# nannau/DoWnGAN

Hardware: AMD Instinct MI355X
Metric: train-step samples/sec (G+D+GP) (higher is better)
Workload: dtype bf16

## Files before the change

### downgan_amd/_lib.py

```python
from __future__ import annotations

import ctypes as C
import os

_HERE = os.path.dirname(os.path.abspath(__file__))
LIB_PATH = os.environ.get("DG_LIB_OVERRIDE") or os.path.join(_HERE, "csrc", "libdowngan_hip.so")

DG_F32, DG_BF16 = 0, 1
STATUS = {0: "DG_OK", -1: "DG_ERR_BAD_SHAPE", -2: "DG_ERR_BAD_DTYPE", -3: "DG_ERR_BAD_ARG", -4: "DG_ERR_LAUNCH"}


class Epilogue(C.Structure):
    _fields_ = [("bias", C.c_void_p), ("has_act", C.c_int), ("act_slope", C.c_float),
                ("r1", C.c_void_p), ("ldr1", C.c_int64), ("s1", C.c_float),
                ("r2", C.c_void_p), ("ldr2", C.c_int64), ("s2", C.c_float),
                ("mask", C.c_void_p), ("ldmask", C.c_int64), ("mask_slope", C.c_float),
                ("accumulate", C.c_int), ("mask_bits", C.c_void_p), ("out_bits", C.c_void_p),
                ("mask_c0", C.c_int), ("mask_last", C.c_int), ("out_q", C.c_void_p), ("out_qs", C.c_void_p), ("ldqs", C.c_int64),
                ("out_u", C.c_void_p), ("out_ue", C.c_void_p), ("skip_y", C.c_int), ("out_amax", C.c_void_p)]


class ConvGeom(C.Structure):
    _fields_ = [("dtype", C.c_int), ("N", C.c_int), ("H", C.c_int), ("W", C.c_int),
                ("Cin", C.c_int), ("Cout", C.c_int), ("stride", C.c_int), ("cin_real", C.c_int), ("pixel_shuffle", C.c_int),
# ... 102 lines not shown
                ("thr", (C.c_float * OBJ_MAX_THR) * HIST_MAX_OUT)]


class DistmapSpec(C.Structure):
    _fields_ = [("speed_u", C.c_int), ("speed_v", C.c_int), ("nthr", C.c_int), ("nring", C.c_int), ("cutoff", C.c_int),
                ("scale", C.c_float * EOF_MAX_C), ("offset", C.c_float * EOF_MAX_C),
                ("thr", (C.c_float * DIST_MAX_THR) * HIST_MAX_OUT)]


class TemporalSpec(C.Structure):
    _fields_ = [("speed_u", C.c_int), ("speed_v", C.c_int), ("nthr", C.c_int), ("ndur", C.c_int), ("nlag", C.c_int),
                ("nbins", C.c_int), ("below", C.c_int * TEMPORAL_MAX_THR), ("lag", C.c_int * TEMPORAL_MAX_LAGS),
                ("scale", C.c_float * EOF_MAX_C), ("offset", C.c_float * EOF_MAX_C),
                ("thr", (C.c_float * TEMPORAL_MAX_THR) * HIST_MAX_OUT), ("lo", (C.c_float * TEMPORAL_MAX_LAGS) * HIST_MAX_OUT),
                ("inv_w", (C.c_float * TEMPORAL_MAX_LAGS) * HIST_MAX_OUT)]


MINMAX_PARTS = 256
_vp, _i, _i64, _f = C.c_void_p, C.c_int, C.c_int64, C.c_float
_PROTOS = {
    "dg_conv3x3_fwd": [C.POINTER(ConvGeom), C.POINTER(Epilogue), _vp, _vp, _vp, _vp],
    "dg_conv3x3_dgrad": [C.POINTER(ConvGeom), C.POINTER(Epilogue), _vp, _vp, _vp, _vp],
    "dg_conv3x3_wgrad": [C.POINTER(ConvGeom), _vp, _vp, _vp, _vp, _vp],
    "dg_conv3x3_wgrad_dense": [_vp, _i, _vp, _vp, _vp, _vp, _vp],
    "dg_conv3x3_wgrad_f8": [C.POINTER(ConvGeom), _vp, _vp, _vp, _vp, _vp, _vp],
    "dg_exp_from_amax": [_vp, _i, _i, _vp, _vp],
    "dg_conv3x3_wgrad_dense_f8": [C.POINTER(ConvGeom), _i, _vp, _vp, _vp, _vp, _vp, _vp],
    "dg_gather_gemm": [C.POINTER(GGDesc), C.POINTER(Epilogue), _vp, _vp, _vp, _vp],
    "dg_conv3x3_plan": [C.POINTER(ConvGeom), _i, C.POINTER(GGDesc)],
    "dg_last_conv_kernels": [],
    "dg_last_wgrad_kernel": [],
    "dg_conv3x3_dgrad_launches": [C.POINTER(ConvGeom)],
    "dg_conv3x3_dgrad_stream_eligible": [C.POINTER(ConvGeom), C.POINTER(Epilogue)],
    "dg_set_s2_dgrad_stream": [C.c_int],
    "dg_colsum": [_i, _vp, _i64, _i64, _i64, _i64, _i, _vp, _vp],
    "dg_colsum_multi": [_i, _vp, _i64, _i64, _i, _i, _vp, _vp],
    "dg_repack_conv_weights": [_i, _i, _vp, _vp, _i, _i, _vp],
    "dg_repack_dense_dgrad": [_i, _vp, _i, _i, _vp, _vp],
    "dg_wgrad_unswap": [_vp, _vp, _i, _i, _vp],
    "dg_linear_fwd": [_i, _vp, _i64, _vp, _i64, _vp, _i, _i, _i, _i64, _vp],
    "dg_linear_dx": [_i, _i, _vp, _i, _vp, _i64, _vp, _i64, _vp, _i64, _f, _i, _i, _i64, _vp],
    "dg_linear_dw": [_i, _vp, _i, _vp, _i64, _vp, _i64, _i, _i, _i64, _vp],
    "dg_linear_dw_wide": [_i, _vp, _i, _vp, _i64, _vp, _i64, _i, _i, _i64, _i, _vp],
    "dg_bias_act": [_i, _vp, _i, _vp, _vp, _i, _i, _i, _i, _f, _vp, _i, _f, _vp],
    "dg_mask_mul": [_i, _vp, _i64, _vp, _i64, _i64, _i, _f, _vp],
    "dg_axpby": [_i, _vp, _i64, _vp, _i64, _f, _vp, _i64, _f, _i64, _i, _vp],
    "dg_gp_interp": [_i, _vp, _vp, _vp, _vp, _i, _i64, _vp],
    "dg_gp_interp_c2": [_i, _vp, _vp, _i64, _vp, _vp, _vp, _vp, _i, _i64, _vp],
    "dg_scale_rows_c2": [_i, _vp, _i64, _vp, _vp, _i, _i64, _vp],
    "dg_sumsq_rows": [_i, _vp, _i, _i64, _vp, _vp],
    "dg_gp_finish": [_vp, _i, _i, _f, _f, _vp, _vp, _vp],
    "dg_scale_rows": [_i, _vp, _vp, _vp, _i, _i64, _vp],
    "dg_l1": [_i, _vp, _i64, _vp, _i64, _i64, _i, _vp, _vp, _i64, _f, _vp, _i64, _vp],
    "dg_sqdiff": [_i, _vp, _i64, _vp, _i64, _i64, _i, _vp, _vp],
    "dg_sum_strided": [_vp, _i, _i, _f, _vp, _vp],
    "dg_fill_col": [_vp, _i, _i, _i, _f, _vp],
    "dg_adam": [_vp, _vp, _vp, _vp, _vp, _i64, _f, _f, _f, _f, _i, _f, _vp],
    "dg_nchw_to_nhwc": [_i, _vp, _vp, _i, _i, _i, _i, _i, _vp],
    "dg_nhwc_to_nchw": [_i, _vp, _i64, _vp, _i, _i, _i, _i, _vp],
    "dg_cast": [_i, _vp, _vp, _i64, _vp],
    "dg_minmax_partial": [_i, _vp, _i64, _i64, _i, _vp, _vp],
    "dg_minmax_finish": [_vp, _i, _vp, _vp],
    "dg_normalise_planar": [_i, _vp, _i, _i, _i, _i64, _i, _vp, _vp, _vp],
    "dg_ssim_level": [_vp, _vp, _i, _i, _i, C.POINTER(SsimParams), _vp, _vp],
    "dg_avgpool2": [_vp, _vp, _i, _i, _i, _vp],
    "dg_msssim_finish": [_vp, _i, _i, C.POINTER(MsssimCombine), _vp, _vp],
    "dg_div_vort_sums": [_i, _vp, _i64, _vp, _i64, _i, _i, _i, _vp, _vp],
# ... 127 lines not shown
```

### downgan_amd/csrc/conv_plan.hip

```cpp
#include "gg_common.h"

thread_local int g_last_kinds = 0;

static int gg_validate(const dg_gg_desc* d, bool f8 = false, bool compact_src = false) {
  if (d->dtype != DG_F32 && d->dtype != DG_BF16) return DG_ERR_BAD_DTYPE;
  const int epc = f8 ? 16 : d->dtype == DG_F32 ? 4 : 8;
  if (d->N <= 0 || d->Hs <= 0 || d->Ws <= 0 || d->Hg <= 0 || d->Wg <= 0 || d->Hd <= 0 || d->Wd <= 0) return DG_ERR_BAD_SHAPE;
  if (d->Cred <= 0 || d->Cred % 8 || d->Nout <= 0 || d->Nout % 16) return DG_ERR_BAD_SHAPE;
  if (d->ntaps < 1 || d->ntaps > 9) return DG_ERR_BAD_SHAPE;
  if ((compact_src ? d->lds % 2 || d->lds < 2 : d->lds % epc) || d->ldd % 4 || d->ldw % epc) return DG_ERR_BAD_SHAPE;
  for (int t = 0; t < d->ntaps; ++t) {
    if (d->tap_dy[t] < -1 || d->tap_dy[t] > 1 || d->tap_dx[t] < -1 || d->tap_dx[t] > 1) return DG_ERR_BAD_ARG;
    if (d->tap_w[t] < 0 || d->tap_w[t] > 8) return DG_ERR_BAD_ARG;
  }
  if (d->src_ps && ((d->Cred / 4) % 8)) return DG_ERR_BAD_SHAPE;
  if (d->dst_ps && ((d->Nout / 4) % 16)) return DG_ERR_BAD_SHAPE;
  if ((long long)d->N * d->Hg * d->Wg >= (1ll << 31)) return DG_ERR_BAD_SHAPE;
  if (d->dst_ps) {
    if (2 * d->Hg > d->Hd || 2 * d->Wg > d->Wd) return DG_ERR_BAD_SHAPE;
  } else {
    if ((d->Hg - 1) * d->dy_mul + d->dy_off >= d->Hd || (d->Wg - 1) * d->dx_mul + d->dx_off >= d->Wd) return DG_ERR_BAD_SHAPE;
    if (d->dy_off < 0 || d->dx_off < 0 || d->dy_mul < 1 || d->dx_mul < 1) return DG_ERR_BAD_SHAPE;
  }
  return DG_OK;
// ... 147 lines not shown
  }
  int nd = 0;
  const int st = g->stride;
  for (int ph = 0; ph < st; ++ph)
    for (int pw = 0; pw < st; ++pw) {
      dg_gg_desc d{};
      d.dtype = g->dtype; d.N = g->N; d.Hs = Ho; d.Ws = Wo; d.Cred = g->Cout; d.lds = g->ldy;
      d.src_ps = g->pixel_shuffle;
      d.Hg = g->H / st; d.Wg = g->W / st; d.sy_mul = 1; d.sx_mul = 1;
      d.ntaps = 0;
      for (int r = 0; r < 3; ++r) {
        if ((ph + 1 - r) % st) continue;
        for (int s = 0; s < 3; ++s) {
          if ((pw + 1 - s) % st) continue;
          d.tap_dy[d.ntaps] = (ph + 1 - r) / st; d.tap_dx[d.ntaps] = (pw + 1 - s) / st;
          d.tap_w[d.ntaps] = r * 3 + s;
          ++d.ntaps;
        }
      }
      d.Nout = g->Cin; d.ldw = 9ll * g->Cout;
      d.Hd = g->H; d.Wd = g->W; d.ldd = g->ldx;
      d.dy_mul = d.dx_mul = st; d.dy_off = ph; d.dx_off = pw; d.dst_ps = 0;
      out[nd++] = d;
    }
  return nd;
}

extern "C" int dg_conv3x3_fwd(const dg_conv_geom* g, const dg_epilogue* ep, const void* x, const void* w_fwd,
                              void* y, void* stream) {
  dg_gg_desc d[4];
  g_last_kinds = 0;
  int n = dg_conv3x3_plan(g, 0, d);
  if (n < 0) return n;
  const bool small = g->cin_real > 0 && g->cin_real <= 2 && g->stride == 1 && !g->pixel_shuffle;
  return gather_gemm_impl(&d[0], ep, x, w_fwd, y, stream, small);
}

static bool seg_dgrad_desc(const dg_gg_desc* d, int n, dg_gg_desc* out) {
  const int epc = d[0].dtype == DG_F32 ? 4 : 8;
  if (n != 4 || d[0].src_ps || d[0].dst_ps || (d[0].Cred / epc) % 8 || d[0].Nout <= 64 || d[0].Hg < 8 || d[0].Wg < 8) return false;
  if (d[0].ntaps != 1 || d[1].ntaps != 2 || d[2].ntaps != 2 || d[3].ntaps != 4) return false;
  if (!gg_halo_row_step_ok(d[0].Ws, d[0].lds, d[0].dtype, 1)) return false;
  *out = d[3];
  out->ntaps = 0;
  for (int c = 0; c < 4; ++c) {
    if (d[c].dy_off != (c >> 1) || d[c].dx_off != (c & 1) || d[c].dy_mul != 2 || d[c].dx_mul != 2) return false;
    for (int t = 0; t < d[c].ntaps; ++t, ++out->ntaps) {
      out->tap_dy[out->ntaps] = d[c].tap_dy[t]; out->tap_dx[out->ntaps] = d[c].tap_dx[t]; out->tap_w[out->ntaps] = d[c].tap_w[t];
    }
  }
  return out->ntaps == 9;
}

extern "C" int dg_conv3x3_dgrad(const dg_conv_geom* g, const dg_epilogue* ep, const void* dy, const void* w_dgrad,
                                void* dx, void* stream) {
  if (g && g->Cin % 16) return DG_ERR_BAD_SHAPE;
  dg_gg_desc d[4];
  g_last_kinds = 0;
  int n = dg_conv3x3_plan(g, 1, d);
  if (n < 0) return n;
  if (s2dgrad_stream_mode() && s2dgrad_stream_eligible(g, ep))
    return s2dgrad_stream_launch(g, ep, dy, w_dgrad, dx, reinterpret_cast<hipStream_t>(stream));
  dg_gg_desc ds;
  if (seg_dgrad_desc(d, n, &ds)) return gather_gemm_impl(&ds, ep, dy, w_dgrad, dx, stream, false, nullptr, true);
  for (int i = 0; i < n; ++i) {
    int rc = dg_gather_gemm(&d[i], ep, dy, w_dgrad, dx, stream);
// ... 9 lines not shown
  int n = dg_conv3x3_plan(g, 0, d);
  if (n < 0) return n;
  d[0].lds = q->ldxq;
  return gather_gemm_impl(&d[0], ep, q->xq, q->wq, y, stream, false, q);
}

extern "C" int dg_conv3x3_dgrad_f8(const dg_conv_geom* g, const dg_epilogue* ep, const dg_f8_operands* q, void* dx, void* stream) {
  if (!q || !g || g->dtype != DG_BF16 || g->pixel_shuffle || g->Cout % 128 || g->Cin % 16) return DG_ERR_BAD_SHAPE;
  dg_gg_desc d[4];
  g_last_kinds = 0;
  int n = dg_conv3x3_plan(g, 1, d);
  if (n < 0) return n;
  dg_gg_desc ds;
  if (seg_dgrad_desc(d, n, &ds) && ds.Cred % 128 == 0) {
    ds.lds = q->ldxq;
    return gather_gemm_impl(&ds, ep, q->xq, q->wq, dx, stream, false, q, true);
  }
  for (int i = 0; i < n; ++i) {
    d[i].lds = q->ldxq;
    int rc = gather_gemm_impl(&d[i], ep, q->xq, q->wq, dx, stream, false, q);
    if (rc) return rc;
  }
  return DG_OK;
}

extern "C" int dg_last_conv_kernels(void) { return g_last_kinds; }

extern "C" int dg_conv3x3_dgrad_stream_eligible(const dg_conv_geom* g, const dg_epilogue* ep) {
  const int rc = geom_validate(g);
  if (rc) return rc;
  return s2dgrad_stream_eligible(g, ep) ? 1 : 0;
}

extern "C" int dg_conv3x3_dgrad_launches(const dg_conv_geom* g) {
  dg_gg_desc d[4], ds;
  const int n = dg_conv3x3_plan(g, 1, d);
  if (n < 0) return n;
  return seg_dgrad_desc(d, n, &ds) ? 1 : n;
}
```

### downgan_amd/csrc/gg_common.h

```cpp
#pragma once
#include "dg_internal.h"

#include <stdlib.h>
#include <type_traits>


extern thread_local int g_last_kinds;

struct GGArgs {
  const void* x; const void* w; void* y;
  const float* bias; const void* r1; const void* r2; const void* mask;
  const void* mask_bits; void* out_bits;
  void* out_q; void* out_qs;
  void* out_u; const unsigned char* out_ue;
  int no_y;
  unsigned* out_amax;
  int ldqs, qs_shift;
  long long ldx, ldw, ldy, ldr1, ldr2, ldmask;
  int M, Hg, Wg, Hs, Ws;
  int cch, kchunks, Cred, ntaps;
  int sy_mul, sx_mul;
  unsigned long long tap_lo; unsigned tap_hi;
  int Nout, Hd, Wd, dy_mul, dx_mul, dy_off, dx_off;
  int src_ps, dst_ps, cps_src_chunks, cps_dst;
// ... 482 lines not shown
      case 2328: run(std::integral_constant<int, 2328>{}, htag); break;
      case 2336: run(std::integral_constant<int, 2336>{}, htag); break;
      case 258: run(std::integral_constant<int, 258>{}, htag); break;
      case 261: run(std::integral_constant<int, 261>{}, htag); break;
      case 2306: run(std::integral_constant<int, 2306>{}, htag); break;
      case 2309: run(std::integral_constant<int, 2309>{}, htag); break;
      case 4353: run(std::integral_constant<int, 4353>{}, htag); break;
      case 4354: run(std::integral_constant<int, 4354>{}, htag); break;
      case 4357: run(std::integral_constant<int, 4357>{}, htag); break;
      case 6402: run(std::integral_constant<int, 6402>{}, htag); break;
      case 6405: run(std::integral_constant<int, 6405>{}, htag); break;
      default: run(std::integral_constant<int, -1>{}, htag); break;
    }
  };
  dispatch(std::integral_constant<int, 0>{});
  EPI_STAMP(2);
  if constexpr (NH == 2) dispatch(std::integral_constant<int, 1>{});
  EPI_STAMP(3);
#undef EPI_STAMP
}

struct F8Args { const unsigned char* xs; const unsigned char* ws; int ldxs; };

int gg_launch_rows(GGArgs& a, int dtype, hipStream_t st);
bool gg_regroup_taps_by_plane(GGArgs& a);
bool gg_halo_row_step_ok(long long Ws, long long ldx, int dtype, int mult);
int gg_launch_halo(GGArgs& a, int dtype, int N, bool s2, bool ps, int nw, hipStream_t st);
int gg_launch_halo_f8(GGArgs& a, const F8Args& f, int N, bool s2, int nw, hipStream_t st);
int gg_launch_halo16(GGArgs& a, int dtype, int N, hipStream_t st);
int gg_launch_im2col(GGArgs& a, int dtype, hipStream_t st);
bool s2dgrad_stream_eligible(const dg_conv_geom* g, const dg_epilogue* ep);
int s2dgrad_stream_mode();
int s2dgrad_stream_launch(const dg_conv_geom* g, const dg_epilogue* ep, const void* dy, const void* w, void* dx, hipStream_t st);
```

### include/downgan_hip.h

```cpp
#ifndef DOWNGAN_HIP_H
#define DOWNGAN_HIP_H

#include <stddef.h>
#include <stdint.h>

#ifdef __cplusplus
extern "C" {
#endif

#define DG_F32 0
#define DG_BF16 1

typedef enum dg_status {
  DG_OK = 0,
  DG_ERR_BAD_SHAPE = -1,
  DG_ERR_BAD_DTYPE = -2,
  DG_ERR_BAD_ARG = -3,
  DG_ERR_LAUNCH = -4
} dg_status;

typedef struct dg_epilogue {
  const float* bias;
  int has_act;
  float act_slope;
// ... 47 lines not shown
                     const void* w_dgrad, void* dx, void* stream);

int dg_conv3x3_wgrad(const dg_conv_geom* g, const void* x, const void* dy, float* dw, float* db,
                     void* stream);

int dg_conv3x3_wgrad_dense(const dg_conv_geom* g, int nconv, const void* x, const void* dy,
                           float* const* dw, float* const* db, void* stream);

int dg_conv3x3_wgrad_f8(const dg_conv_geom* g, const void* xq, const void* ex, const void* dyq, const void* ey, float* dw,
                        void* stream);

int dg_conv3x3_wgrad_dense_f8(const dg_conv_geom* g, int nconv, const void* xq, const void* ex, const void* dyq, const void* ey,
                              float* const* dw, void* stream);

int dg_colsum(int dtype, const void* dy, int64_t rows_outer, int64_t ld_outer, int64_t rows_inner,
              int64_t ld, int C, float* db, void* stream);

int dg_colsum_multi(int dtype, const void* dy, int64_t rows, int64_t ld, int C, int nseg, float* const* db, void* stream);

int dg_gather_gemm(const dg_gg_desc* d, const dg_epilogue* ep, const void* x, const void* w, void* y,
                   void* stream);

int dg_last_conv_kernels(void);

int dg_last_wgrad_kernel(void);

int dg_conv3x3_plan(const dg_conv_geom* g, int kind, dg_gg_desc* out);

int dg_conv3x3_dgrad_launches(const dg_conv_geom* g);

int dg_conv3x3_dgrad_stream_eligible(const dg_conv_geom* g, const dg_epilogue* ep);

int dg_set_s2_dgrad_stream(int on);

int dg_repack_conv_weights(int dtype, int kind, const float* master, void* dst, int CoutP, int CinP,
                           void* stream);
int dg_repack_dense_dgrad(int dtype, const float* const* masters, int nconv, int F, void* dst, void* stream);
int dg_wgrad_unswap(const float* tmp, float* dw, int CoutP, int CinP, void* stream);


int dg_linear_fwd(int dtype, const void* x, int64_t ldx, const void* w, int64_t ldw, float* y,
                  int ldy, int B, int O, int64_t K, void* stream);
int dg_linear_dx(int dtype, int out_dtype, const float* dy, int ldo, const void* w, int64_t ldw,
                 void* dx, int64_t lddx, const void* mask, int64_t ldmask, float mask_slope, int B,
                 int O, int64_t K, void* stream);
int dg_linear_dw(int dtype, const float* dy, int ldo, const void* x, int64_t ldx, float* dw,
                 int64_t lddw, int B, int O, int64_t K, void* stream);
int dg_linear_dw_wide(int dtype, const float* dy, int ldo, const void* x, int64_t ldx, float* dw,
                      int64_t lddw, int B, int O, int64_t K, int accumulate, void* stream);


int dg_bias_act(int out_dtype, const float* in, int ldi, const float* bias, void* out, int ldo,
                int rows, int C, int has_act, float slope, const void* mask, int ldmask,
                float mask_slope, void* stream);
int dg_mask_mul(int dtype, void* u, int64_t ldu, const void* y, int64_t ldy, int64_t rows, int C,
                float slope, void* stream);
int dg_axpby(int dtype, void* out, int64_t ldo, const void* x, int64_t ldx, float a, const void* y,
             int64_t ldy, float b, int64_t rows, int C, void* stream);
int dg_gp_interp(int dtype, const void* real, const void* fake, const float* alpha, void* xhat,
                 int B, int64_t per_img, void* stream);
int dg_gp_interp_c2(int dtype, const void* real, const void* fake, int64_t ld, const float* alpha,
                    void* xhat_c, void* real_c, void* fake_c, int B, int64_t pix_per_img, void* stream);
int dg_scale_rows_c2(int dtype, const void* g, int64_t ld, const float* coef, void* out_c, int B,
                     int64_t pix_per_img, void* stream);
int dg_sumsq_rows(int dtype, const void* g, int B, int64_t per_img, float* ss, void* stream);
int dg_gp_finish(const float* ss, int B, int B_global, float gp_lambda, float weight, float* coef,
// ... 283 lines not shown
```

Baseline: 74.25.

## Add persistent warp-specialized streaming kernel for stride-2 128-channel conv forward

```diff
diff --git a/downgan_amd/_lib.py b/downgan_amd/_lib.py
--- a/downgan_amd/_lib.py
+++ b/downgan_amd/_lib.py
@@ -159,6 +159,8 @@
     "dg_conv3x3_dgrad_launches": [C.POINTER(ConvGeom)],
     "dg_conv3x3_dgrad_stream_eligible": [C.POINTER(ConvGeom), C.POINTER(Epilogue)],
     "dg_set_s2_dgrad_stream": [C.c_int],
+    "dg_conv3x3_fwd_stream_eligible": [C.POINTER(ConvGeom), C.POINTER(Epilogue)],
+    "dg_set_s2_fwd_stream": [C.c_int],
     "dg_colsum": [_i, _vp, _i64, _i64, _i64, _i64, _i, _vp, _vp],
     "dg_colsum_multi": [_i, _vp, _i64, _i64, _i, _i, _vp, _vp],
     "dg_repack_conv_weights": [_i, _i, _vp, _vp, _i, _i, _vp],
diff --git a/downgan_amd/csrc/conv_plan.hip b/downgan_amd/csrc/conv_plan.hip
--- a/downgan_amd/csrc/conv_plan.hip
+++ b/downgan_amd/csrc/conv_plan.hip
@@ -203,6 +203,8 @@
   g_last_kinds = 0;
   int n = dg_conv3x3_plan(g, 0, d);
   if (n < 0) return n;
+  if (s2fwd_stream_mode() && s2fwd_stream_eligible(g, ep))
+    return s2fwd_stream_launch(g, ep, x, w_fwd, y, reinterpret_cast<hipStream_t>(stream));
   const bool small = g->cin_real > 0 && g->cin_real <= 2 && g->stride == 1 && !g->pixel_shuffle;
   return gather_gemm_impl(&d[0], ep, x, w_fwd, y, stream, small);
 }
@@ -278,6 +280,12 @@
   return s2dgrad_stream_eligible(g, ep) ? 1 : 0;
 }
 
+extern "C" int dg_conv3x3_fwd_stream_eligible(const dg_conv_geom* g, const dg_epilogue* ep) {
+  const int rc = geom_validate(g);
+  if (rc) return rc;
+  return s2fwd_stream_eligible(g, ep) ? 1 : 0;
+}
+
 extern "C" int dg_conv3x3_dgrad_launches(const dg_conv_geom* g) {
   dg_gg_desc d[4], ds;
   const int n = dg_conv3x3_plan(g, 1, d);
diff --git a/downgan_amd/csrc/conv_s2fwd.hip b/downgan_amd/csrc/conv_s2fwd.hip
--- /dev/null
+++ b/downgan_amd/csrc/conv_s2fwd.hip
@@ -0,0 +1,306 @@
+#include "gg_common.h"
+
+#ifndef S2F_ABL
+#define S2F_ABL 0
+#endif
+
+namespace {
+
+constexpr int NT = 512;
+constexpr int PITCH = 288;
+constexpr int ODD_PIX = 17, EVEN_PIX = 16;
+constexpr int EVEN_OFF = ODD_PIX * PITCH;
+constexpr int RING_ROW = (ODD_PIX + EVEN_PIX) * PITCH;
+constexpr int ROW_PIECES = RING_ROW / 16;
+constexpr int NSLOT = 14;
+constexpr int PF = 4;
+static_assert(2 * PF + 5 <= NSLOT, "the requested rows must not land on rows still being read");
+constexpr int NDMA = 5;
+constexpr int HAND_OFF = NSLOT * RING_ROW;
+constexpr int HAND_SLOT = 4 * 64 * 32;
+constexpr int MASK_OFF = HAND_OFF + 2 * HAND_SLOT;
+constexpr int MASK_SLOT = 16 * 16;
+constexpr int LDS_BYTES = MASK_OFF + 2 * MASK_SLOT;
+
+struct S2FArgs {
+  const char* x; const char* w; char* y;
+  char* bits;
+  float slope;
+  int H, W, Ho, Wo;
+  int nstrips, nitems, trips;
+};
+
+__device__ __forceinline__ __amdgpu_buffer_rsrc_t uniform_rsrc(const char* p) {
+  const unsigned long long b = (unsigned long long)p;
+  const unsigned long long u = ((unsigned long long)(unsigned)__builtin_amdgcn_readfirstlane((int)(unsigned)(b >> 32)) << 32) |
+                               (unsigned)__builtin_amdgcn_readfirstlane((int)(unsigned)b);
+  return __builtin_amdgcn_make_buffer_rsrc((void*)u, 0, (int)DG_OOB_OFF, 0x00020000);
+}
+
+template <int EP, bool HEAD>
+__device__ __forceinline__ void s2f_run(const S2FArgs& a, char* lds) {
+  constexpr int NTAP = HEAD ? 5 : 4;
+  const int tid = threadIdx.x, lane = tid & 63, q = (tid >> 6) & 3;
+  const int l15 = lane & 15, g = lane >> 4;
+
+  u32x4_t wr[NTAP * 8];
+  {
+    constexpr int TWH[5] = {4, 3, 5, 1, 7}, TWT[4] = {0, 2, 6, 8};
+#pragma unroll
+    for (int t = 0; t < NTAP; ++t)
+#pragma unroll
+      for (int cb = 0; cb < 2; ++cb)
+#pragma unroll
+        for (int kk = 0; kk < 2; ++kk)
+#pragma unroll
+          for (int j = 0; j < 2; ++j) {
+            const int n = 32 * q + 8 * (l15 >> 2) + 4 * j + (l15 & 3);
+            const int tw = HEAD ? TWH[t] : TWT[t];
+            wr[((t * 2 + cb) * 2 + kk) * 2 + j] =
+                *reinterpret_cast<const u32x4_t*>(a.w + ((long long)n * 1152 + tw * 128 + 64 * cb + 32 * kk + 8 * g) * 2);
+          }
+#pragma unroll
+    for (int i = 0; i < NTAP * 8; ++i) asm volatile("" : "+v"(wr[i]));
+  }
+  const char* const fb0 = lds + l15 * PITCH + g * 16;
+  auto wrap = [](int v) { return v >= NSLOT ? v - NSLOT : v; };
+  auto frag = [&](int slot, int s, int cb, int kk) {
+    return *reinterpret_cast<const uint4*>(fb0 + slot * RING_ROW + (s == 1 ? EVEN_OFF : s == 2 ? PITCH : 0) + cb * 128 + kk * 64);
+  };
+  auto tap = [&](int t, int cb, int slot, int s, f32x4_t (&acc)[2]) {
+#pragma unroll
+    for (int kk = 0; kk < 2; ++kk) {
+      const uint4 b = frag(slot, s, cb, kk);
+#pragma unroll
+      for (int j = 0; j < 2; ++j) {
+        if (S2F_ABL & 4) acc[j][0] += __uint_as_float(b.x ^ wr[((t * 2 + cb) * 2 + kk) * 2 + j][0]);
+        else Mma<bf16_t>::run(__builtin_bit_cast(uint4, wr[((t * 2 + cb) * 2 + kk) * 2 + j]), b, acc[j]);
+      }
+    }
+  };
+  char* const hand = lds + HAND_OFF + q * (64 * 32) + lane * 32;
+
+  if constexpr (HEAD) {
+    const int hw = __builtin_amdgcn_readfirstlane(tid >> 6) - 4;
+    int dsrc[NDMA], ddst[NDMA];
+    unsigned dpad = 0, dfirst = 0;
+#pragma unroll
+    for (int m = 0; m < NDMA; ++m) {
+      int i = hw + 4 * m;
+      if (i > 18) i = 18;
+      ddst[m] = i < 18 ? i * 1024 : 2 * RING_ROW - 1024;
+      const int P = ddst[m] / 16 + lane, rs = P >= ROW_PIECES ? 1 : 0, Pr = P - ROW_PIECES * rs, ps = Pr / 18, c = Pr - 18 * ps;
+      const int pi = ps < ODD_PIX ? 2 * ps : 2 * (ps - ODD_PIX) + 1;
+      dsrc[m] = (rs * a.W + pi - 1) * 256 + c * 16;
+      if (c >= 16) dpad |= 1u << m;
+      if (pi == 0) dfirst |= 1u << m;
+    }
+    const int ring_m0 = __builtin_amdgcn_readfirstlane((int)(unsigned long long)((__attribute__((address_space(3))) char*)lds));
+    const int htid = tid - 256;
+
+    for (int trip = 0; trip < a.trips; ++trip) {
+      const int item = (int)blockIdx.x + trip * (int)gridDim.x;
+      if (item >= a.nitems) break;
+      const int img = item / a.nstrips, x0 = (item - img * a.nstrips) * 16;
+      typedef int i32x4h_t __attribute__((ext_vector_type(4)));
+      i32x4h_t rs4;
+      {
+        const unsigned long long xb = (unsigned long long)(a.x + (long long)img * a.H * a.W * 256);
+        rs4[0] = __builtin_amdgcn_readfirstlane((int)(unsigned)xb);
+        rs4[1] = __builtin_amdgcn_readfirstlane((int)(unsigned)(xb >> 32) & 0xffff);
+        rs4[2] = (int)DG_OOB_OFF;
+        rs4[3] = 0x00020000;
+      }
+      unsigned doff[NDMA];
+#pragma unroll
+      for (int m = 0; m < NDMA; ++m)
+        doff[m] = (((dpad >> m) & 1u) || (x0 == 0 && ((dfirst >> m) & 1u))) ? DG_OOB_OFF : (unsigned)(dsrc[m] + 2 * x0 * 256);
+      auto request_pair = [&](int row, int slot) {
+        const bool ok = row < a.H && !(S2F_ABL & 2);
+        const unsigned ro = (unsigned)row * (unsigned)a.W * 256u;
+#pragma unroll
+        for (int m = 0; m < NDMA; ++m) {
+          const unsigned off = ok ? doff[m] + ro : DG_OOB_OFF;
+          asm volatile("s_mov_b32 m0, %0\n\ts_nop 0\n\tbuffer_load_dwordx4 %1, %2, 0 offen lds"
+                       :: "s"(ring_m0 + slot * RING_ROW + ddst[m]), "v"(off), "s"(rs4) : "memory");
+        }
+      };
+      asm volatile("s_waitcnt vmcnt(0)" ::: "memory");
+#pragma unroll
+      for (int z = 0; z < 3; ++z)
+        if (htid + 256 * z < ROW_PIECES) *reinterpret_cast<uint4*>(lds + (NSLOT - 1) * RING_ROW + (htid + 256 * z) * 16) = uint4{0u, 0u, 0u, 0u};
+      if (x0 == 0 && htid < NSLOT * 16) *reinterpret_cast<uint4*>(lds + (htid >> 4) * RING_ROW + (htid & 15) * 16) = uint4{0u, 0u, 0u, 0u};
+#pragma unroll
+      for (int d = 0; d < PF; ++d) request_pair(2 * d, 2 * d);
+      asm volatile("s_waitcnt vmcnt(%0)" :: "n"(NDMA * (PF - 1)) : "memory");
+      __syncthreads();
+      int sk = 0;
+      for (int k = 0; k <= a.Ho; ++k) {
+        request_pair(2 * (k + PF), wrap(sk + 2 * PF));
+        if (k < a.Ho) {
+          const int sM = wrap(sk + NSLOT - 1), sP = sk + 1;
+          f32x4_t acc[2] = {f32x4_t{0.f, 0.f, 0.f, 0.f}, f32x4_t{0.f, 0.f, 0.f, 0.f}};
+#pragma unroll
+          for (int cb = 0; cb < 2; ++cb) tap(0, cb, sk, 1, acc);
+#pragma unroll
+          for (int cb = 0; cb < 2; ++cb) { tap(1, cb, sk, 0, acc); tap(2, cb, sk, 2, acc); }
+#pragma unroll
+          for (int cb = 0; cb < 2; ++cb) { tap(3, cb, sM, 1, acc); tap(4, cb, sP, 1, acc); }
+          char* const h = hand + (k & 1) * HAND_SLOT;
+          *reinterpret_cast<f32x4_t*>(h) = acc[0];
+          *reinterpret_cast<f32x4_t*>(h + 16) = acc[1];
+        }
+        asm volatile("s_waitcnt vmcnt(%0)" :: "n"(NDMA * (PF - 1)) : "memory");
+        __syncthreads();
+        sk = wrap(sk + 2);
+      }
+    }
+  } else {
+    const bool mwave = EP == 1 && __builtin_amdgcn_readfirstlane(tid >> 6) == 0;
+    const unsigned st_lane = (unsigned)(l15 * 256 + 64 * q + 16 * g);
+
+    for (int trip = 0; trip < a.trips; ++trip) {
+      const int item = (int)blockIdx.x + trip * (int)gridDim.x;
+      if (item >= a.nitems) break;
+      const int img = item / a.nstrips, x0 = (item - img * a.nstrips) * 16;
+      const __amdgpu_buffer_rsrc_t rY = uniform_rsrc(a.y + (long long)img * a.Ho * a.Wo * 256);
+      const __amdgpu_buffer_rsrc_t rB = uniform_rsrc(a.bits + (long long)img * a.Ho * a.Wo * 16);
+      const unsigned mfill_off = (mwave && lane < 16) ? (unsigned)((x0 + lane) * 16) : DG_OOB_OFF;
+      auto fetch_mask = [&](int R) {
+        return __builtin_amdgcn_raw_buffer_load_b128(rB, R < a.Ho ? mfill_off + (unsigned)R * (unsigned)a.Wo * 16u : DG_OOB_OFF, 0, 0);
+      };
+      const char* const mrd = lds + MASK_OFF + l15 * 16 + 4 * q + g;
+      u32x4_t ms0 = {0u, 0u, 0u, 0u}, ms1 = {0u, 0u, 0u, 0u};
+      if (mwave) ms0 = fetch_mask(0);
+      __syncthreads();
+
+      auto step = [&](int k, int sk, const u32x4_t& mstaged, u32x4_t& mnxt) __attribute__((always_inline)) {
+        if (mwave) mnxt = fetch_mask(k + 1);
+        if (k > 0) {
+          const int R = k - 1;
+          const char* const h = hand + (R & 1) * HAND_SLOT;
+          f32x4_t acc[2] = {*reinterpret_cast<const f32x4_t*>(h), *reinterpret_cast<const f32x4_t*>(h + 16)};
+          unsigned mb = 0;
+          if (EP == 1) mb = *reinterpret_cast<const unsigned char*>(mrd + (R & 1) * MASK_SLOT);
+          const int sM = wrap(sk + NSLOT - 3), sP = wrap(sk + NSLOT - 1);
+#pragma unroll
+          for (int cb = 0; cb < 2; ++cb) {
+            tap(0, cb, sM, 0, acc); tap(1, cb, sM, 2, acc); tap(2, cb, sP, 0, acc); tap(3, cb, sP, 2, acc);
+          }
+          float v[8] = {acc[0][0], acc[0][1], acc[0][2], acc[0][3], acc[1][0], acc[1][1], acc[1][2], acc[1][3]};
+          const unsigned pix = (unsigned)R * (unsigned)a.Wo + (unsigned)x0;
+          if (EP == 0) {
+            if (a.slope >= 0.f && a.slope <= 1.f) {
+              typedef float f32x2_t __attribute__((ext_vector_type(2)));
+              const f32x2_t sl2 = {a.slope, a.slope};
+#pragma unroll
+              for (int e = 0; e < 8; e += 2) {
+                const f32x2_t p = f32x2_t{v[e], v[e + 1]} * sl2;
+                v[e] = __builtin_fmaxf(v[e], p[0]); v[e + 1] = __builtin_fmaxf(v[e + 1], p[1]);
+              }
+            } else {
+#pragma unroll
+              for (int e = 0; e < 8; ++e) v[e] = leaky(v[e], a.slope);
+            }
+          } else {
+            unsigned sh = mb << 24;
+            const float one = 1.f;
+#pragma unroll
+            for (int e = 7; e >= 0; --e) {
+              float f;
+              asm("v_add_co_u32_e32 %1, vcc, %1, %1\n\tv_cndmask_b32_e32 %0, %2, %3, vcc" : "=&v"(f), "+v"(sh) : "v"(a.slope), "v"(one) : "vcc");
+              v[e] *= f;
+            }
+          }
+          u32x4_t t;
+#pragma unroll
+          for (int e = 0; e < 4; ++e) t[e] = pack_bf16x2(v[2 * e], v[2 * e + 1]);
+          __builtin_amdgcn_raw_buffer_store_b128(t, rY, (S2F_ABL & 1) ? DG_OOB_OFF : pix * 256u + st_lane, 0, 0);
+          if (EP == 0) {
+            unsigned ob = 0;
+#pragma unroll
+            for (int e = 7; e >= 0; --e)
+              asm("v_cmp_lt_f32_e32 vcc, 0, %1\n\tv_addc_co_u32_e32 %0, vcc, %0, %0, vcc" : "+v"(ob) : "v"(v[e]) : "vcc");
+            ob <<= 8 * g;
+            ob |= (unsigned)__shfl_xor((int)ob, 16, 64);
+            ob |= (unsigned)__shfl_xor((int)ob, 32, 64);
+            __builtin_amdgcn_raw_buffer_store_b32(ob, rB, (g == 0 && !(S2F_ABL & 1)) ? (pix + (unsigned)l15) * 16u + 4u * q : DG_OOB_OFF, 0, 0);
+          }
+        }
+        if (mwave && lane < 16) *reinterpret_cast<uint4*>(lds + MASK_OFF + (k & 1) * MASK_SLOT + lane * 16) = __builtin_bit_cast(uint4, mstaged);
+        __syncthreads();
+      };
+      int sk = 0;
+      for (int k = 0; k <= a.Ho; k += 2) {
+        step(k, sk, ms0, ms1);
+        sk = wrap(sk + 2);
+        if (k + 1 <= a.Ho) { step(k + 1, sk, ms1, ms0); sk = wrap(sk + 2); }
+      }
+    }
+  }
+}
+
+std::atomic<int> g_s2f_stream{1};
+std::atomic<int> g_cus{0};
+
+}
+
+template <int EP>
+__global__ __launch_bounds__(NT, 1) void s2fwd_stream_kernel(const S2FArgs a) {
+  extern __shared__ __attribute__((aligned(16))) char s2f_lds[];
+  if (__builtin_amdgcn_readfirstlane(threadIdx.x >> 6) < 4) s2f_run<EP, false>(a, s2f_lds);
+  else s2f_run<EP, true>(a, s2f_lds);
+}
+
+bool s2fwd_stream_eligible(const dg_conv_geom* g, const dg_epilogue* ep) {
+  if (!g || !ep || g->dtype != DG_BF16 || g->stride != 2 || g->pixel_shuffle) return false;
+  if (g->N <= 0 || g->H <= 0 || g->W <= 0 || ((g->H | g->W) & 1)) return false;
+  if (g->Cin != 128 || g->Cout != 128 || g->ldx != 128 || g->ldy != 128) return false;
+  if ((g->W / 2) % 16) return false;
+  if (!gg_halo_row_step_ok(g->W, g->ldx, g->dtype, 2)) return false;
+  if ((long long)g->H * g->W * 256 >= (1ll << 31)) return false;
+  if (ep->bias || ep->r1 || ep->r2 || ep->mask || ep->accumulate || ep->mask_c0 || ep->mask_last || ep->out_q || ep->out_qs || ep->out_u ||
+      ep->out_ue || ep->skip_y || ep->out_amax)
+    return false;
+  const bool act_bits = ep->has_act && ep->out_bits && !ep->mask_bits;
+  const bool tangent = !ep->has_act && !ep->out_bits && ep->mask_bits;
+  return act_bits || tangent;
+}
+
+int s2fwd_stream_mode() { return g_s2f_stream.load(std::memory_order_relaxed); }
+
+extern "C" int dg_set_s2_fwd_stream(int on) { return g_s2f_stream.exchange(on < 0 ? 0 : on, std::memory_order_relaxed); }
+
+int s2fwd_stream_launch(const dg_conv_geom* g, const dg_epilogue* ep, const void* x, const void* w, void* y, hipStream_t st) {
+  if (!x || !w || !y || !ep) return DG_ERR_BAD_ARG;
+  int cus = g_cus.load(std::memory_order_relaxed);
+  if (cus <= 0) {
+    int dev = 0;
+    if (hipGetDevice(&dev) != hipSuccess || hipDeviceGetAttribute(&cus, hipDeviceAttributeMultiprocessorCount, dev) != hipSuccess || cus <= 0)
+      return DG_ERR_LAUNCH;
+    g_cus.store(cus, std::memory_order_relaxed);
+  }
+  const bool act_bits = ep->has_act != 0;
+  S2FArgs a{};
+  a.x = (const char*)x; a.w = (const char*)w; a.y = (char*)y;
+  a.bits = act_bits ? (char*)ep->out_bits : (char*)const_cast<void*>(ep->mask_bits);
+  a.slope = act_bits ? ep->act_slope : ep->mask_slope;
+  a.H = g->H; a.W = g->W; a.Ho = g->H / 2; a.Wo = g->W / 2;
+  a.nstrips = a.Wo / 16;
+  const long long items = (long long)g->N * a.nstrips;
+  if (items >= (1ll << 31)) return DG_ERR_BAD_SHAPE;
+  a.nitems = (int)items;
+  const int mode = s2fwd_stream_mode();
+  int grid = mode > 1 && mode < cus ? mode : cus;
+  if (grid > a.nitems) grid = a.nitems;
+  a.trips = (a.nitems + grid - 1) / grid;
+  g_last_kinds |= 128;
+  if (act_bits) {
+    DG_SET_MAX_LDS_ONCE((&s2fwd_stream_kernel<0>), LDS_BYTES);
+    hipLaunchKernelGGL(s2fwd_stream_kernel<0>, dim3(grid), dim3(NT), LDS_BYTES, st, a);
+  } else {
+    DG_SET_MAX_LDS_ONCE((&s2fwd_stream_kernel<1>), LDS_BYTES);
+    hipLaunchKernelGGL(s2fwd_stream_kernel<1>, dim3(grid), dim3(NT), LDS_BYTES, st, a);
+  }
+  return dg_check_launch();
+}
diff --git a/downgan_amd/csrc/gg_common.h b/downgan_amd/csrc/gg_common.h
--- a/downgan_amd/csrc/gg_common.h
+++ b/downgan_amd/csrc/gg_common.h
@@ -538,3 +538,6 @@
 bool s2dgrad_stream_eligible(const dg_conv_geom* g, const dg_epilogue* ep);
 int s2dgrad_stream_mode();
 int s2dgrad_stream_launch(const dg_conv_geom* g, const dg_epilogue* ep, const void* dy, const void* w, void* dx, hipStream_t st);
+bool s2fwd_stream_eligible(const dg_conv_geom* g, const dg_epilogue* ep);
+int s2fwd_stream_mode();
+int s2fwd_stream_launch(const dg_conv_geom* g, const dg_epilogue* ep, const void* x, const void* w, void* y, hipStream_t st);
diff --git a/include/downgan_hip.h b/include/downgan_hip.h
--- a/include/downgan_hip.h
+++ b/include/downgan_hip.h
@@ -103,6 +103,10 @@
 int dg_conv3x3_dgrad_stream_eligible(const dg_conv_geom* g, const dg_epilogue* ep);
 
 int dg_set_s2_dgrad_stream(int on);
+
+int dg_conv3x3_fwd_stream_eligible(const dg_conv_geom* g, const dg_epilogue* ep);
+
+int dg_set_s2_fwd_stream(int on);
 
 int dg_repack_conv_weights(int dtype, int kind, const float* master, void* dst, int CoutP, int CinP,
                            void* stream);
```

After: 74.57, median of 6. Within noise of the previous version (+0.4%).

## Add persistent streaming kernel for stride-2 128-channel conv forward

Applied to the files above, without the earlier changes.

```diff
diff --git a/downgan_amd/_lib.py b/downgan_amd/_lib.py
--- a/downgan_amd/_lib.py
+++ b/downgan_amd/_lib.py
@@ -158,7 +158,9 @@
     "dg_last_wgrad_kernel": [],
     "dg_conv3x3_dgrad_launches": [C.POINTER(ConvGeom)],
     "dg_conv3x3_dgrad_stream_eligible": [C.POINTER(ConvGeom), C.POINTER(Epilogue)],
+    "dg_conv3x3_fwd_stream_eligible": [C.POINTER(ConvGeom), C.POINTER(Epilogue)],
     "dg_set_s2_dgrad_stream": [C.c_int],
+    "dg_set_s2_fwd_stream": [C.c_int],
     "dg_colsum": [_i, _vp, _i64, _i64, _i64, _i64, _i, _vp, _vp],
     "dg_colsum_multi": [_i, _vp, _i64, _i64, _i, _i, _vp, _vp],
     "dg_repack_conv_weights": [_i, _i, _vp, _vp, _i, _i, _vp],
diff --git a/downgan_amd/csrc/conv_plan.hip b/downgan_amd/csrc/conv_plan.hip
--- a/downgan_amd/csrc/conv_plan.hip
+++ b/downgan_amd/csrc/conv_plan.hip
@@ -203,6 +203,8 @@
   g_last_kinds = 0;
   int n = dg_conv3x3_plan(g, 0, d);
   if (n < 0) return n;
+  if (const int mode = s2fwd_stream_mode(); mode && s2fwd_stream_eligible(g, ep) && (mode > 1 || s2fwd_stream_items(g) >= S2FWD_STREAM_MIN_ITEMS))
+    return s2fwd_stream_launch(g, ep, x, w_fwd, y, reinterpret_cast<hipStream_t>(stream));
   const bool small = g->cin_real > 0 && g->cin_real <= 2 && g->stride == 1 && !g->pixel_shuffle;
   return gather_gemm_impl(&d[0], ep, x, w_fwd, y, stream, small);
 }
@@ -278,6 +280,12 @@
   return s2dgrad_stream_eligible(g, ep) ? 1 : 0;
 }
 
+extern "C" int dg_conv3x3_fwd_stream_eligible(const dg_conv_geom* g, const dg_epilogue* ep) {
+  const int rc = geom_validate(g);
+  if (rc) return rc;
+  return s2fwd_stream_eligible(g, ep) ? 1 : 0;
+}
+
 extern "C" int dg_conv3x3_dgrad_launches(const dg_conv_geom* g) {
   dg_gg_desc d[4], ds;
   const int n = dg_conv3x3_plan(g, 1, d);
diff --git a/downgan_amd/csrc/conv_s2fwd.hip b/downgan_amd/csrc/conv_s2fwd.hip
--- /dev/null
+++ b/downgan_amd/csrc/conv_s2fwd.hip
@@ -0,0 +1,310 @@
+#include "gg_common.h"
+
+#ifndef DG_S2F_ABL
+#define DG_S2F_ABL 0
+#endif
+#ifndef DG_S2F_ORDER
+#define DG_S2F_ORDER 0
+#endif
+
+namespace {
+
+constexpr int NT = 512;
+constexpr int RING_PIX = 33;
+constexpr int RING_PITCH = 272;
+constexpr int RING_ROW = RING_PIX * RING_PITCH;
+constexpr int RING_SLOTS = 8;
+constexpr int HAND_OFF = RING_SLOTS * RING_ROW;
+constexpr int HAND_BYTES = 2 * 4 * 2 * 64 * 16;
+constexpr int BITS_OFF = HAND_OFF + HAND_BYTES;
+constexpr int LDS_BYTES = BITS_OFF + 2 * 256;
+
+struct S2FArgs {
+  const char* x; const char* w; char* y; const char* mask_bits; char* out_bits;
+  float slope;
+  int H, W, Ho, Wo;
+  int nstrips, nitems, trips;
+};
+
+__device__ __forceinline__ __amdgpu_buffer_rsrc_t uniform_rsrc(const char* p) {
+  const unsigned long long b = (unsigned long long)p;
+  const unsigned long long u = ((unsigned long long)(unsigned)__builtin_amdgcn_readfirstlane((int)(unsigned)(b >> 32)) << 32) |
+                               (unsigned)__builtin_amdgcn_readfirstlane((int)(unsigned)b);
+  return __builtin_amdgcn_make_buffer_rsrc((void*)u, 0, (int)DG_OOB_OFF, 0x00020000);
+}
+
+struct Stage { u32x4_t a0, a1, b0, b1, h, m; };
+
+template <bool ACT>
+__device__ __forceinline__ unsigned store_pixel(const f32x4_t& f0, const f32x4_t& f1, unsigned mb, float slope, __amdgpu_buffer_rsrc_t rY,
+                                                unsigned off) {
+  float v[8] = {f0[0], f0[1], f0[2], f0[3], f1[0], f1[1], f1[2], f1[3]};
+  unsigned ob = 0;
+  if (ACT) {
+    if (slope >= 0.f && slope <= 1.f) {
+      typedef float f32x2_t __attribute__((ext_vector_type(2)));
+      const f32x2_t sl2 = {slope, slope};
+#pragma unroll
+      for (int k = 0; k < 8; k += 2) {
+        const f32x2_t p = f32x2_t{v[k], v[k + 1]} * sl2;
+        v[k] = __builtin_fmaxf(v[k], p[0]); v[k + 1] = __builtin_fmaxf(v[k + 1], p[1]);
+      }
+    } else {
+#pragma unroll
+      for (int k = 0; k < 8; ++k) v[k] = leaky(v[k], slope);
+    }
+  } else {
+    unsigned sh = mb << 24;
+    const float one = 1.f;
+#pragma unroll
+    for (int e = 7; e >= 0; --e) {
+      float f;
+      asm("v_add_co_u32_e32 %1, vcc, %1, %1\n\tv_cndmask_b32_e32 %0, %2, %3, vcc" : "=&v"(f), "+v"(sh) : "v"(slope), "v"(one) : "vcc");
+      v[e] *= f;
+    }
+  }
+  u32x4_t t;
+#pragma unroll
+  for (int k = 0; k < 4; ++k) t[k] = pack_bf16x2(v[2 * k], v[2 * k + 1]);
+  __builtin_amdgcn_raw_buffer_store_b128(t, rY, off, 0, 0);
+  if (ACT) {
+#pragma unroll
+    for (int k = 7; k >= 0; --k)
+      asm("v_cmp_lt_f32_e32 vcc, 0, %1\n\tv_addc_co_u32_e32 %0, vcc, %0, %0, vcc" : "+v"(ob) : "v"(v[k]) : "vcc");
+  }
+  return ob;
+}
+
+template <bool ACT, bool GA>
+__device__ __forceinline__ void s2f_run(const S2FArgs& a, char* lds) {
+  constexpr int NTAP = GA ? 5 : 4;
+  constexpr int TWA[5] = {4, 3, 5, 1, 7}, TROWA[5] = {0, 0, 0, -1, 1}, TCOLA[5] = {1, 0, 2, 1, 1};
+  constexpr int TWB[4] = {0, 2, 6, 8}, TROWB[4] = {-1, -1, 1, 1}, TCOLB[4] = {0, 2, 0, 2};
+  constexpr int NP = GA ? 10 : 8;
+  constexpr int CTA[10] = {0, 0, 1, 2, 1, 2, 3, 4, 3, 4}, CCA[10] = {0, 1, 0, 0, 1, 1, 0, 0, 1, 1};
+  constexpr int CTB[8] = {0, 1, 2, 3, 0, 1, 2, 3}, CCB[8] = {0, 0, 0, 0, 1, 1, 1, 1};
+  const int tid = threadIdx.x, lane = tid & 63, q = (tid >> 6) & 3;
+  const int wave = __builtin_amdgcn_readfirstlane(tid >> 6);
+  const int l15 = lane & 15, g = lane >> 4;
+
+  u32x4_t wr[NTAP * 8];
+#pragma unroll
+  for (int t = 0; t < NTAP; ++t)
+#pragma unroll
+    for (int cb = 0; cb < 2; ++cb)
+#pragma unroll
+      for (int kk = 0; kk < 2; ++kk)
+#pragma unroll
+        for (int j = 0; j < 2; ++j) {
+          const int n = 32 * q + 8 * (l15 >> 2) + 4 * j + (l15 & 3);
+          const int tw = GA ? TWA[t] : TWB[t];
+          wr[((t * 2 + cb) * 2 + kk) * 2 + j] =
+              *reinterpret_cast<const u32x4_t*>(a.w + ((long long)n * 1152 + tw * 128 + 64 * cb + 32 * kk + 8 * g) * 2);
+        }
+#pragma unroll
+  for (int i = 0; i < NTAP * 8; ++i) asm volatile("" : "+v"(wr[i]));
+
+  const int W = a.W, Wo = a.Wo;
+  const char* const fb0 = lds + 2 * l15 * RING_PITCH + g * 16;
+  const int tb = tid & 255;
+  char* const fill_dst = lds + (1 + (tb >> 4)) * RING_PITCH + (tb & 15) * 16;
+  char* const halo_dst = lds + (lane & 15) * 16;
+  const bool owave = ACT && !GA && wave == 4;
+  const bool hwave = GA && wave == 0;
+  const bool mwave = !ACT && GA && wave == 1;
+  char* const hand = lds + HAND_OFF + (q * 2) * 1024 + lane * 16;
+  char* const bits = lds + BITS_OFF;
+
+  for (int trip = 0; trip < a.trips; ++trip) {
+    const int item = (int)(DG_S2F_ORDER ? xcd_remap(blockIdx.x, gridDim.x) : blockIdx.x) + trip * (int)gridDim.x;
+    if (item >= a.nitems) break;
+    const int img = item / a.nstrips, x0 = (item - img * a.nstrips) * 16;
+    const __amdgpu_buffer_rsrc_t rX = uniform_rsrc(a.x + ((long long)img * a.H * W + 2 * x0 - 1) * 256);
+    const __amdgpu_buffer_rsrc_t rY = uniform_rsrc(a.y + ((long long)img * a.Ho * Wo + x0) * 256);
+    const __amdgpu_buffer_rsrc_t rB =
+        uniform_rsrc((ACT ? (const char*)a.out_bits : a.mask_bits) + ((long long)img * a.Ho * Wo + x0) * 16);
+    const unsigned fill_off0 = !(DG_S2F_ABL & 4) && 2 * x0 + (tb >> 4) < W ? 256u + (unsigned)tb * 16u : DG_OOB_OFF;
+    const unsigned fill_off1 = !(DG_S2F_ABL & 4) && 2 * x0 + 16 + (tb >> 4) < W ? 256u + 4096u + (unsigned)tb * 16u : DG_OOB_OFF;
+    const unsigned halo_off = (!(DG_S2F_ABL & 4) && hwave && x0 > 0 && lane < 32) ? (unsigned)(lane & 15) * 16u : DG_OOB_OFF;
+    const unsigned pix_ok = (!(DG_S2F_ABL & 1) && x0 + l15 < Wo) ? 0u : DG_OOB_OFF;
+    const unsigned st_lane = pix_ok | (unsigned)(l15 * 256 + 64 * q + 16 * g);
+    const unsigned bits_lane = (!(DG_S2F_ABL & (ACT ? 1 : 4)) && (ACT ? owave : mwave) && lane < 16 && x0 + lane < Wo) ? (unsigned)lane * 16u : DG_OOB_OFF;
+    const unsigned rowb = (unsigned)W * 256u;
+    auto fetch_piece = [&](unsigned off, int rr) {
+      return __builtin_amdgcn_raw_buffer_load_b128(rX, (rr >= 0 && rr < a.H) ? off + (unsigned)rr * rowb : DG_OOB_OFF, 0, 0);
+    };
+    auto fetch = [&](int j, Stage& s) __attribute__((always_inline)) {
+      if constexpr (GA) {
+        s.h = fetch_piece(halo_off, 2 * j + 2 + ((lane >> 4) & 1));
+        if constexpr (!ACT)
+          s.m = __builtin_amdgcn_raw_buffer_load_b128(rB, (j >= 0 && j < a.Ho) ? bits_lane + (unsigned)j * (unsigned)Wo * 16u : DG_OOB_OFF, 0, 0);
+      } else {
+        s.a0 = fetch_piece(fill_off0, 2 * j + 2);
+        s.a1 = fetch_piece(fill_off1, 2 * j + 2);
+        s.b0 = fetch_piece(fill_off0, 2 * j + 3);
+        s.b1 = fetch_piece(fill_off1, 2 * j + 3);
+      }
+    };
+    auto slot = [](int rr) { return ((rr + 1) & (RING_SLOTS - 1)) * RING_ROW; };
+    auto put = [&](int j, const Stage& s) __attribute__((always_inline)) {
+      const int ra = 2 * j + 2;
+      if constexpr (GA) {
+        if (hwave && lane < 32) *reinterpret_cast<uint4*>(halo_dst + slot(ra + (lane >> 4))) = __builtin_bit_cast(uint4, s.h);
+        if (mwave && lane < 16 && j >= 0) *reinterpret_cast<uint4*>(bits + ((j + 1) & 1) * 256 + lane * 16) = __builtin_bit_cast(uint4, s.m);
+      } else {
+        *reinterpret_cast<uint4*>(fill_dst + slot(ra)) = __builtin_bit_cast(uint4, s.a0);
+        *reinterpret_cast<uint4*>(fill_dst + slot(ra) + 16 * RING_PITCH) = __builtin_bit_cast(uint4, s.a1);
+        *reinterpret_cast<uint4*>(fill_dst + slot(ra + 1)) = __builtin_bit_cast(uint4, s.b0);
+        *reinterpret_cast<uint4*>(fill_dst + slot(ra + 1) + 16 * RING_PITCH) = __builtin_bit_cast(uint4, s.b1);
+      }
+    };
+    Stage S0, S1, S2;
+    fetch(-1, S0);
+    fetch(0, S1);
+    fetch(1, S2);
+    {
+      const uint4 z = {0u, 0u, 0u, 0u};
+      if constexpr (GA) {
+        if (hwave && lane < 16) *reinterpret_cast<uint4*>(halo_dst + slot(-1)) = z;
+      } else {
+        *reinterpret_cast<uint4*>(fill_dst + slot(-1)) = z;
+        *reinterpret_cast<uint4*>(fill_dst + slot(-1) + 16 * RING_PITCH) = z;
+      }
+    }
+    put(-1, S0);
+    __syncthreads();
+
+    auto tick = [&](int k, Stage& ld, const Stage& wr_) __attribute__((always_inline)) {
+      fetch(k + 2, ld);
+      const int y = GA ? k : k - 1;
+      f32x4_t acc[2] = {f32x4_t{0.f, 0.f, 0.f, 0.f}, f32x4_t{0.f, 0.f, 0.f, 0.f}};
+      unsigned mb = 0;
+      if constexpr (!GA) {
+        if (owave && k >= 2 && k - 2 < a.Ho) {
+          const u32x4_t ow = __builtin_bit_cast(u32x4_t, *reinterpret_cast<const uint4*>(bits + ((k - 1) & 1) * 256 + (lane & 15) * 16));
+          __builtin_amdgcn_raw_buffer_store_b128(ow, rB, bits_lane + (unsigned)(k - 2) * (unsigned)Wo * 16u, 0, 0);
+        }
+      }
+      if (GA ? k < a.Ho : (k >= 1 && k <= a.Ho)) {
+        auto rd = [&](int p, uint4 (&b)[2]) {
+          const int t = GA ? CTA[p] : CTB[p], cb = GA ? CCA[p] : CCB[p];
+          const char* const src = fb0 + slot(2 * y + (GA ? TROWA[t] : TROWB[t])) + (GA ? TCOLA[t] : TCOLB[t]) * RING_PITCH + cb * 128;
+          b[0] = *reinterpret_cast<const uint4*>(src);
+          b[1] = *reinterpret_cast<const uint4*>(src + 64);
+        };
+        uint4 b[NP][2];
+        rd(0, b[0]); rd(1, b[1]);
+        if constexpr (!GA) {
+          const char* const h = hand + (y & 1) * 8192;
+          acc[0] = *reinterpret_cast<const f32x4_t*>(h);
+          acc[1] = *reinterpret_cast<const f32x4_t*>(h + 1024);
+          if (!ACT) mb = *reinterpret_cast<const unsigned char*>(bits + (k & 1) * 256 + l15 * 16 + 4 * q + g);
+        }
+#pragma unroll
+        for (int p = 0; p < NP; p += 2) {
+          if (p + 2 < NP) { rd(p + 2, b[p + 2]); rd(p + 3, b[p + 3]); }
+          __builtin_amdgcn_sched_barrier(0);
+#pragma unroll
+          for (int pp = p; pp < p + 2; ++pp) {
+            const int t = GA ? CTA[pp] : CTB[pp], cb = GA ? CCA[pp] : CCB[pp];
+#pragma unroll
+            for (int kk = 0; kk < 2; ++kk)
+#pragma unroll
+              for (int j = 0; j < 2; ++j) {
+                if (DG_S2F_ABL & 2) asm volatile("" :: "v"(b[pp][kk].x), "v"(b[pp][kk].y), "v"(b[pp][kk].z), "v"(b[pp][kk].w));
+                else Mma<bf16_t>::run(__builtin_bit_cast(uint4, wr[((t * 2 + cb) * 2 + kk) * 2 + j]), b[pp][kk], acc[j]);
+              }
+          }
+          __builtin_amdgcn_sched_barrier(0);
+        }
+        if constexpr (GA) {
+          char* const h = hand + (k & 1) * 8192;
+          *reinterpret_cast<f32x4_t*>(h) = acc[0];
+          *reinterpret_cast<f32x4_t*>(h + 1024) = acc[1];
+        } else {
+          const unsigned ob = store_pixel<ACT>(acc[0], acc[1], mb, a.slope, rY, st_lane + (unsigned)y * (unsigned)Wo * 256u);
+          if (ACT) *reinterpret_cast<unsigned char*>(bits + (k & 1) * 256 + l15 * 16 + 4 * q + g) = (unsigned char)ob;
+        }
+      }
+      put(k, wr_);
+      __syncthreads();
+    };
+    const int T = a.Ho + 1;
+    int k = 0;
+    for (; k < T; k += 3) {
+      tick(k, S0, S1);
+      tick(k + 1, S1, S2);
+      tick(k + 2, S2, S0);
+    }
+    if (owave && k == T) {
+      const u32x4_t ow = __builtin_bit_cast(u32x4_t, *reinterpret_cast<const uint4*>(bits + (a.Ho & 1) * 256 + (lane & 15) * 16));
+      __builtin_amdgcn_raw_buffer_store_b128(ow, rB, bits_lane + (unsigned)(a.Ho - 1) * (unsigned)Wo * 16u, 0, 0);
+    }
+  }
+}
+
+std::atomic<int> g_s2f_stream{1};
+std::atomic<int> g_s2f_cus{0};
+
+}
+
+template <bool ACT>
+__global__ __launch_bounds__(NT, 1) void s2fwd_stream_kernel(const S2FArgs a) {
+  extern __shared__ __attribute__((aligned(16))) char s2f_lds[];
+  if (__builtin_amdgcn_readfirstlane(threadIdx.x >> 6) < 4) s2f_run<ACT, true>(a, s2f_lds);
+  else s2f_run<ACT, false>(a, s2f_lds);
+}
+
+bool s2fwd_stream_eligible(const dg_conv_geom* g, const dg_epilogue* ep) {
+  if (!g || !ep || g->dtype != DG_BF16 || g->stride != 2 || g->pixel_shuffle) return false;
+  if (g->N <= 0 || g->H <= 0 || g->W <= 0 || ((g->H | g->W) & 1)) return false;
+  if (g->Cin != 128 || g->Cout != 128 || g->ldx != 128 || g->ldy != 128) return false;
+  if (!gg_halo_row_step_ok(g->W, g->ldx, g->dtype, 2)) return false;
+  if ((long long)g->H * g->W * 256 >= (1ll << 31)) return false;
+  if (ep->bias || ep->r1 || ep->r2 || ep->mask || ep->accumulate || ep->mask_c0 || ep->mask_last || ep->out_q || ep->out_qs || ep->out_u ||
+      ep->out_ue || ep->skip_y || ep->out_amax)
+    return false;
+  const bool form_a = ep->has_act && ep->out_bits && !ep->mask_bits;
+  const bool form_b = ep->mask_bits && !ep->has_act && !ep->out_bits;
+  return form_a || form_b;
+}
+
+long long s2fwd_stream_items(const dg_conv_geom* g) { return (long long)g->N * ((g->W / 2 + 15) / 16); }
+
+int s2fwd_stream_mode() { return g_s2f_stream.load(std::memory_order_relaxed); }
+
+extern "C" int dg_set_s2_fwd_stream(int mode) { return g_s2f_stream.exchange(mode < 0 ? 0 : mode, std::memory_order_relaxed); }
+
+int s2fwd_stream_launch(const dg_conv_geom* g, const dg_epilogue* ep, const void* x, const void* w, void* y, hipStream_t st) {
+  if (!x || !w || !y || !ep) return DG_ERR_BAD_ARG;
+  int cus = g_s2f_cus.load(std::memory_order_relaxed);
+  if (cus <= 0) {
+    int dev = 0;
+    if (hipGetDevice(&dev) != hipSuccess || hipDeviceGetAttribute(&cus, hipDeviceAttributeMultiprocessorCount, dev) != hipSuccess || cus <= 0)
+      return DG_ERR_LAUNCH;
+    g_s2f_cus.store(cus, std::memory_order_relaxed);
+  }
+  const bool act = ep->has_act != 0;
+  S2FArgs a{};
+  a.x = (const char*)x; a.w = (const char*)w; a.y = (char*)y;
+  a.mask_bits = (const char*)ep->mask_bits; a.out_bits = (char*)ep->out_bits;
+  a.slope = act ? ep->act_slope : ep->mask_slope;
+  a.H = g->H; a.W = g->W; a.Ho = g->H / 2; a.Wo = g->W / 2;
+  a.nstrips = (a.Wo + 15) / 16;
+  const long long items = s2fwd_stream_items(g);
+  if (items >= (1ll << 31)) return DG_ERR_BAD_SHAPE;
+  a.nitems = (int)items;
+  const int mode = s2fwd_stream_mode();
+  int grid = mode > 1 && mode < cus ? mode : cus;
+  if (grid > a.nitems) grid = a.nitems;
+  a.trips = (a.nitems + grid - 1) / grid;
+  g_last_kinds |= 128;
+  if (act) {
+    DG_SET_MAX_LDS_ONCE((&s2fwd_stream_kernel<true>), LDS_BYTES);
+    hipLaunchKernelGGL(s2fwd_stream_kernel<true>, dim3(grid), dim3(NT), LDS_BYTES, st, a);
+  } else {
+    DG_SET_MAX_LDS_ONCE((&s2fwd_stream_kernel<false>), LDS_BYTES);
+    hipLaunchKernelGGL(s2fwd_stream_kernel<false>, dim3(grid), dim3(NT), LDS_BYTES, st, a);
+  }
+  return dg_check_launch();
+}
diff --git a/downgan_amd/csrc/gg_common.h b/downgan_amd/csrc/gg_common.h
--- a/downgan_amd/csrc/gg_common.h
+++ b/downgan_amd/csrc/gg_common.h
@@ -538,3 +538,8 @@
 bool s2dgrad_stream_eligible(const dg_conv_geom* g, const dg_epilogue* ep);
 int s2dgrad_stream_mode();
 int s2dgrad_stream_launch(const dg_conv_geom* g, const dg_epilogue* ep, const void* dy, const void* w, void* dx, hipStream_t st);
+constexpr long long S2FWD_STREAM_MIN_ITEMS = 256;
+bool s2fwd_stream_eligible(const dg_conv_geom* g, const dg_epilogue* ep);
+long long s2fwd_stream_items(const dg_conv_geom* g);
+int s2fwd_stream_mode();
+int s2fwd_stream_launch(const dg_conv_geom* g, const dg_epilogue* ep, const void* x, const void* w, void* y, hipStream_t st);
diff --git a/include/downgan_hip.h b/include/downgan_hip.h
--- a/include/downgan_hip.h
+++ b/include/downgan_hip.h
@@ -103,6 +103,10 @@
 int dg_conv3x3_dgrad_stream_eligible(const dg_conv_geom* g, const dg_epilogue* ep);
 
 int dg_set_s2_dgrad_stream(int on);
+
+int dg_conv3x3_fwd_stream_eligible(const dg_conv_geom* g, const dg_epilogue* ep);
+
+int dg_set_s2_fwd_stream(int mode);
 
 int dg_repack_conv_weights(int dtype, int kind, const float* master, void* dst, int CoutP, int CinP,
                            void* stream);
```

After: 73.82 before, 74.05 after (median of 6 runs). About the same (+0.3%).
